# FordyceLab/magnify

Measured on AMD Instinct MI355X. Metric: megapixels/sec through flatfield+segment+ROI-reduce; markers/sec, higher is better.
Workload: dtype u16

## Files before the change

magnify_amd/csrc/mg_circles.hip:

```cpp
#include <math.h>
#include <stdlib.h>

#include "mg_common.h"

namespace {

constexpr int NT = 256;

constexpr uint64_t GOLDEN = 0x9E3779B97F4A7C15ull;
__device__ __forceinline__ uint64_t mix64(uint64_t z) {
  z ^= z >> 30;
  z *= 0xBF58476D1CE4E5B9ull;
  z ^= z >> 27;
  z *= 0x94D049BB133111EBull;
  return z ^ (z >> 31);
}
__device__ __forceinline__ uint32_t mix_top32(uint64_t z) { return (uint32_t)(mix64(z) >> 32); }

__device__ __forceinline__ uint32_t div_f64(double x, double d, double inv_d) {
  uint32_t q = (uint32_t)(x * inv_d);
  const double r = fma(-(double)q, d, x);
  if (r < 0.0) --q;
  else if (r >= d) ++q;
  return q;
}

__device__ __forceinline__ uint64_t div_u64(uint64_t n, uint64_t d, double inv_d) {
  uint64_t q = (uint64_t)((double)n * inv_d);
  int64_t r = (int64_t)(n - q * d);
  if (r < 0) {
    --q;
    r += (int64_t)d;
  }
  if (r >= (int64_t)d) ++q;
  return q;
}

constexpr double BISECTOR_EPS = (double)1e-20f;
__device__ __forceinline__ double2 bisector(int d_row, int d_col) {
  const double m = (double)(-d_col) / ((double)d_row + BISECTOR_EPS);
  return make_double2(m, 0.5 * (double)d_row - m * (0.5 * (double)d_col));
}

struct DivFull {
  __device__ __forceinline__ double operator()(double num, double den) const { return num / den; }
};
struct DivUnscaled {
  __device__ __forceinline__ double operator()(double num, double den) const {
    if (!(fabs(den) > 0.0 && fabs(den) < 1.0e300)) return num / den;
    double y = __builtin_amdgcn_rcp(den);
    double e = fma(-den, y, 1.0);
    y = fma(y, e, y);
    e = fma(-den, y, 1.0);
    y = fma(y, e, y);
    double q = num * y;
    const double r = fma(-den, q, num);
    return fma(r, y, q);
  }
};

template <class Div>
__device__ __forceinline__ float3 circle_from_bisectors(double2 l1, double2 l2, int p0r, int p0c, Div div) {
  const float c_col = (float)div(l1.y - l2.y, l2.x - l1.x + BISECTOR_EPS);
  const float c_row = (float)(l1.x * (double)c_col + l1.y);
  const float rad = sqrtf(c_row * c_row + c_col * c_col);
  return make_float3((float)((double)c_row + (double)p0r), (float)((double)c_col + (double)p0c), rad);
}

__device__ __forceinline__ void store_raw(float* __restrict__ d_raw, int64_t index, float3 c) {
  if (!d_raw) return;
  float* o = d_raw + index * 3;
  o[0] = c.x;
  o[1] = c.y;
  o[2] = c.z;
}

template <class Emit>
__device__ __forceinline__ void candidate_cell(float3 c, int h, int w, int min_r, int max_r, int ntc, Emit&& emit) {
  if (!(c.z >= (float)min_r && c.z <= (float)max_r)) return;
  const float rr = rintf(c.x), rc = rintf(c.y);
  if (!(fabsf(rr) < 1.0e9f && fabsf(rc) < 1.0e9f)) return;
  const int ir = (int)rr, ic = (int)rc, irad = (int)rintf(c.z);
  if (ir + irad < 0 || ic + irad < 0 || ir - irad >= h || ic - irad >= w) return;
  const int pr = ir + max_r, pc = ic + max_r;
  emit((pr >> 6) * ntc + (pc >> 6), irad - min_r, pr & 63, pc & 63);
}

template <bool FAST>
__global__ __launch_bounds__(NT) void k_candidates(const int32_t* __restrict__ d_coords, int64_t coord_cap,
                                                   const int32_t* __restrict__ d_starts,
                                                   const int32_t* __restrict__ d_counts,
                                                   const int32_t* __restrict__ d_num_edges, int h, int w, int grid,
                                                   int gc, int n_cells, const uint64_t* __restrict__ d_seeds,
                                                   int64_t num_iter, int min_r, int max_r,
                                                   uint32_t* __restrict__ d_bitmap, int64_t bitmap_words,
                                                   float* __restrict__ d_raw, uint32_t* __restrict__ d_keys) {
  const int plane = blockIdx.y;
  const uint32_t n_edges = (uint32_t)d_num_edges[plane];
  if (n_edges == 0) return;
  const int32_t* coords = d_coords + (int64_t)plane * coord_cap * 2;
  const int32_t* starts = d_starts + (int64_t)plane * n_cells;
  const int32_t* counts = d_counts + (int64_t)plane * n_cells;
  const uint64_t seed = d_seeds[plane];
  const int ntc = (w + 2 * max_r + 63) >> 6, nr = max_r - min_r + 1;
  uint32_t* bitmap = d_bitmap ? d_bitmap + (int64_t)plane * bitmap_words : nullptr;
  uint32_t* keys = d_keys ? d_keys + (int64_t)plane * num_iter : nullptr;
  const double inv_iter = 1.0 / (double)num_iter;
  const int64_t it0 = (int64_t)blockIdx.x * NT + threadIdx.x, stride = (int64_t)gridDim.x * NT;
  uint64_t zbase = seed + ((uint64_t)it0 * 3ull + 1ull) * GOLDEN;
  const uint64_t zstep = (uint64_t)stride * 3ull * GOLDEN;
  const uint32_t eq = FAST ? n_edges / (uint32_t)num_iter : 0u;
  const double er = FAST ? (double)(n_edges - eq * (uint32_t)num_iter) : 0.0, dk = (double)num_iter;
  const uint32_t gmagic = grid > 1 ? 0xFFFFFFFFu / (uint32_t)grid + 1u : 0u;
  for (int64_t it = it0; it < num_iter; it += stride, zbase += zstep) {
    uint64_t sa, sb;
    if (FAST) {
      const double x = (double)(uint32_t)it * er;
      sa = (uint64_t)((uint32_t)it * eq + div_f64(x, dk, inv_iter));
      sb = (uint64_t)(((uint32_t)it + 1u) * eq + div_f64(x + er, dk, inv_iter));
    } else {
      sa = div_u64((uint64_t)it * n_edges, (uint64_t)num_iter, inv_iter);
      sb = div_u64(((uint64_t)it + 1) * n_edges, (uint64_t)num_iter, inv_iter);
    }
    const uint64_t width = sb > sa ? sb - sa : 1;
    const uint32_t u0 = (uint32_t)(sa + (((uint64_t)mix_top32(zbase) * width) >> 32));
    const int p0r = coords[2 * (int64_t)u0], p0c = coords[2 * (int64_t)u0 + 1];
    const int cell = FAST ? (int)(__umulhi((uint32_t)p0r, gmagic) * (uint32_t)gc + __umulhi((uint32_t)p0c, gmagic))
                           : (p0r / grid) * gc + (p0c / grid);
    const uint32_t cnt = (uint32_t)counts[cell];
    const int64_t base = starts[cell];
    const uint64_t z12 = mix64(zbase + GOLDEN);
    const int64_t i1 = base + (int64_t)__umulhi((uint32_t)(z12 >> 32), cnt);
    const int64_t i2 = base + (int64_t)__umulhi((uint32_t)z12, cnt);
    const double2 l1 = bisector(coords[2 * i1] - p0r, coords[2 * i1 + 1] - p0c);
    const double2 l2 = bisector(coords[2 * i2] - p0r, coords[2 * i2 + 1] - p0c);
    const float3 c = circle_from_bisectors(l1, l2, p0r, p0c, DivFull{});
    store_raw(d_raw, (int64_t)plane * num_iter + it, c);
    uint32_t key = MG_NO_KEY;
    candidate_cell(c, h, w, min_r, max_r, ntc, [&](int tile, int layer, int row, int col) {
      if (keys) {
        key = mg_key_pack(tile, layer, row, col);
      } else {
        const int64_t bit = (((int64_t)tile * nr + layer) << 12) + (row << 6) + col;
        atomicOr(&bitmap[bit >> 5], 1u << (bit & 31));
      }
    });
    if (keys) keys[it] = key;
  }
}

constexpr int CT = 1024;
constexpr int MAX_TAB_GRID = 32;

__global__ __launch_bounds__(CT) void k_candidates_tab(const int32_t* __restrict__ d_coords, int64_t coord_cap,
                                                       const int32_t* __restrict__ d_starts,
                                                       const int32_t* __restrict__ d_counts,
                                                       const int32_t* __restrict__ d_num_edges, int h, int w, int grid,
                                                       int gc, int n_cells, const uint64_t* __restrict__ d_seeds,
                                                       uint32_t num_iter, int min_r, int max_r,
                                                       float* __restrict__ d_raw, uint32_t* __restrict__ d_keys) {
  extern __shared__ double2 s_tab[];
  const int plane = blockIdx.y;
  const uint32_t n_edges = (uint32_t)d_num_edges[plane];
  if (n_edges == 0) return;
  const int g1 = grid - 1, span = 2 * grid - 1;
  for (int i = threadIdx.x; i < span * span; i += CT) s_tab[i] = bisector(i / span - g1, i - (i / span) * span - g1);
  __syncthreads();
  const int32_t* coords = d_coords + (int64_t)plane * coord_cap * 2;
  const int32_t* starts = d_starts + (int64_t)plane * n_cells;
  const int32_t* counts = d_counts + (int64_t)plane * n_cells;
  const uint64_t seed = d_seeds[plane];
  const int ntc = (w + 2 * max_r + 63) >> 6;
  uint32_t* keys = d_keys ? d_keys + (int64_t)plane * num_iter : nullptr;
  const uint32_t K = num_iter;
  const uint32_t it0 = blockIdx.x * CT + threadIdx.x, stride = gridDim.x * CT;
  if (it0 >= K) return;
  const uint32_t eq = n_edges / K, er = n_edges - eq * K;
  const double inv_k = 1.0 / (double)K;
  const uint64_t x0 = (uint64_t)it0 * er;
  const uint64_t q0 = div_u64(x0, K, inv_k);
  uint32_t sa = it0 * eq + (uint32_t)q0, rem = (uint32_t)(x0 - q0 * K);
  const uint64_t xs = (uint64_t)stride * er;
  const uint64_t qs = div_u64(xs, K, inv_k);
  const uint32_t sa_step = stride * eq + (uint32_t)qs, rem_step = (uint32_t)(xs - qs * K);
  uint64_t zbase = seed + ((uint64_t)it0 * 3ull + 1ull) * GOLDEN;
  const uint64_t zstep = (uint64_t)stride * 3ull * GOLDEN;
  const uint32_t gmagic = 0xFFFFFFFFu / (uint32_t)grid + 1u;
  for (uint32_t it = it0; it < K; it += stride, zbase += zstep) {
    const uint32_t sb = sa + eq + (rem + er >= K ? 1u : 0u);
    uint32_t u0 = sa;
    if (sb > sa + 1u) u0 = sa + __umulhi(mix_top32(zbase), sb - sa);
    {
      const uint32_t t = rem + rem_step;
      const bool carry = t >= K;
      sa += sa_step + (carry ? 1u : 0u);
      rem = carry ? t - K : t;
    }
    const int2 p0 = reinterpret_cast<const int2*>(coords)[u0];
    const int p0r = p0.x, p0c = p0.y;
    const int cell = (int)(__umulhi((uint32_t)p0r, gmagic) * (uint32_t)gc + __umulhi((uint32_t)p0c, gmagic));
    const uint32_t cnt = (uint32_t)counts[cell];
    const uint32_t base = (uint32_t)starts[cell];
    const uint64_t z12 = mix64(zbase + GOLDEN);
    const uint32_t i1 = base + __umulhi((uint32_t)(z12 >> 32), cnt);
    const uint32_t i2 = base + __umulhi((uint32_t)z12, cnt);
    const int2 p1 = reinterpret_cast<const int2*>(coords)[i1], p2 = reinterpret_cast<const int2*>(coords)[i2];
    const int d1r = p1.x - p0r, d1c = p1.y - p0c, d2r = p2.x - p0r, d2c = p2.y - p0c;
    double2 l1, l2;
    if ((uint32_t)(d1r + g1) < (uint32_t)span && (uint32_t)(d1c + g1) < (uint32_t)span &&
        (uint32_t)(d2r + g1) < (uint32_t)span && (uint32_t)(d2c + g1) < (uint32_t)span) {
      l1 = s_tab[(d1r + g1) * span + d1c + g1], l2 = s_tab[(d2r + g1) * span + d2c + g1];
    } else {
      l1 = bisector(d1r, d1c), l2 = bisector(d2r, d2c);
    }
    const float3 c = circle_from_bisectors(l1, l2, p0r, p0c, DivUnscaled{});
    store_raw(d_raw, ((int64_t)plane * num_iter + it), c);
    uint32_t key = MG_NO_KEY;
    candidate_cell(c, h, w, min_r, max_r, ntc, [&](int tile, int layer, int row, int col) { key = mg_key_pack(tile, layer, row, col); });
    if (keys) keys[it] = key;
  }
}

constexpr int TS = 64;
constexpr int LAYER_WORDS = 128;

__global__ __launch_bounds__(NT) void k_layer_count(const uint32_t* __restrict__ d_bitmap, int64_t bitmap_words,
                                                    int n_layers, int32_t* __restrict__ d_layer_offsets) {
  const int plane = blockIdx.y;
  const int layer = blockIdx.x * (NT / 64) + (threadIdx.x >> 6);
  if (layer >= n_layers) return;
  const int lane = threadIdx.x & 63;
  const uint2 v = reinterpret_cast<const uint2*>(d_bitmap + (int64_t)plane * bitmap_words +
                                                 (int64_t)layer * LAYER_WORDS)[lane];
  const int c = mg_wave_sum_i32(__popc(v.x) + __popc(v.y));
  if (lane == 0) d_layer_offsets[(int64_t)plane * (n_layers + 1) + layer] = c;
}

constexpr int MAX_RANGES = 64;
constexpr int DEDUP_TX = 2;

template <int TX>
__global__ __launch_bounds__(NT) void k_tile_dedup(const uint32_t* __restrict__ d_keys, int64_t num_iter,
                                                   const int32_t* __restrict__ d_starts,
                                                   const int32_t* __restrict__ d_counts,
                                                   const int32_t* __restrict__ d_num_edges, int h, int w, int grid,
                                                   int gr, int gc, int ntc, int nr, int max_r,
                                                   uint32_t* __restrict__ d_ukeys, int64_t circle_cap,
                                                   int32_t* __restrict__ d_tile_ranges, int n_tiles,
                                                   int32_t* __restrict__ d_num_circles,
                                                   int32_t* __restrict__ d_layer_starts) {
  extern __shared__ uint32_t lbits[];
  __shared__ long long s_lo[MAX_RANGES];
  __shared__ int s_pre[MAX_RANGES + 1];
  __shared__ int s_cnt[TX * 32 + 1];
  __shared__ int s_base;
  const int plane = blockIdx.z, tr = blockIdx.y, tc0 = blockIdx.x * TX;
  const int ntx = min(TX, ntc - tc0);
  const int tile0 = tr * ntc + tc0;
  const int words = nr * LAYER_WORDS;
  for (int i = threadIdx.x; i < ntx * words; i += NT) lbits[i] = 0u;
  const long long n_edges = d_num_edges[plane];
  const int reach = max_r + 2;
  const int y0 = max(tr * TS - max_r - reach, 0), y1 = min(tr * TS + TS - 1 - max_r + reach, h - 1);
  const int x0 = max(tc0 * TS - max_r - reach, 0), x1 = min((tc0 + ntx) * TS - 1 - max_r + reach, w - 1);
  int n_ranges = 0;
  if (n_edges > 0 && y0 <= y1 && x0 <= x1) {
    const int cr0 = y0 / grid, cr1 = y1 / grid, cc0 = x0 / grid, cc1 = x1 / grid;
    n_ranges = cr1 - cr0 + 1;
    if ((int)threadIdx.x < n_ranges) {
      const int32_t* starts = d_starts + (int64_t)plane * gr * gc;
      const int32_t* counts = d_counts + (int64_t)plane * gr * gc;
      const int cr = cr0 + threadIdx.x;
      const long long ea = starts[cr * gc + cc0], eb = (long long)starts[cr * gc + cc1] + counts[cr * gc + cc1];
      long long lo = 0, hi = 0;
      if (eb > ea) {
        const double kpe = (double)num_iter / (double)n_edges;
        hi = min((long long)((double)eb * kpe) + 3, (long long)num_iter);
        lo = min(max((long long)((double)ea * kpe) - 2, 0ll), hi);
      }
      s_lo[threadIdx.x] = lo;
      s_pre[threadIdx.x + 1] = (int)(hi - lo);
    }
  }
  __syncthreads();
  if (threadIdx.x == 0) {
    s_pre[0] = 0;
    for (int r = 0; r < n_ranges; ++r) s_pre[r + 1] += s_pre[r];
  }
  __syncthreads();
  const uint32_t* keys = d_keys + (int64_t)plane * num_iter;
  constexpr int KB = 8;
  for (int r = 0; r < n_ranges; ++r) {
    const uint32_t* kr = keys + s_lo[r];
    const int len = s_pre[r + 1] - s_pre[r];
    for (int base = threadIdx.x; base < len; base += NT * KB) {
      uint32_t kv[KB];
#pragma unroll
      for (int u = 0; u < KB; ++u) {
        const int i = base + u * NT;
        kv[u] = i < len ? kr[i] : MG_NO_KEY;
      }
#pragma unroll
      for (int u = 0; u < KB; ++u) {
        const uint32_t key = kv[u];
        const uint32_t t = mg_key_tile(key) - (uint32_t)tile0;
        if (t < (uint32_t)ntx) atomicOr(&lbits[t * words + (mg_key_low17(key) >> 5)], 1u << (key & 31u));
      }
    }
  }
  __syncthreads();
  const int n_li = ntx * nr;
  const int n_words = n_li * LAYER_WORDS;
  const int per = (n_words + NT - 1) / NT;
  const int w0 = min((int)threadIdx.x * per, n_words), w1 = min(w0 + per, n_words);
  int mine = 0;
  for (int wd = w0; wd < w1; ++wd) mine += __popc(lbits[wd]);
  int n_unique;
  const int ex = mg_block_exscan(mine, &n_unique);
  {
    int run = ex;
    for (int wd = w0; wd < w1; ++wd) {
      if ((wd & (LAYER_WORDS - 1)) == 0) s_cnt[wd / LAYER_WORDS] = run;
      run += __popc(lbits[wd]);
    }
  }
  if (threadIdx.x == 0) {
    s_cnt[n_li] = n_unique;
    s_base = n_unique ? atomicAdd(&d_num_circles[plane], n_unique) : 0;
  }
  __syncthreads();
  const int64_t base = s_base;
  if ((int)threadIdx.x < ntx) {
    int32_t* tr2 = d_tile_ranges + ((int64_t)plane * n_tiles + tile0 + threadIdx.x) * 2;
    tr2[0] = (int32_t)min(base + s_cnt[threadIdx.x * nr], circle_cap);
    tr2[1] = s_cnt[(threadIdx.x + 1) * nr] - s_cnt[threadIdx.x * nr];
  }
  if (d_layer_starts) {
    for (int i = threadIdx.x; i < ntx * (nr + 1); i += NT) {
      const int t = i / (nr + 1), ri = i - t * (nr + 1);
      d_layer_starts[((int64_t)plane * n_tiles + tile0 + t) * (nr + 1) + ri] =
          (int32_t)min(base + s_cnt[t * nr + ri], circle_cap);
    }
  }
  uint32_t* out = d_ukeys + (int64_t)plane * circle_cap;
  int64_t pos = base + ex;
  for (int wd = w0; wd < w1; ++wd) {
    uint32_t bits = lbits[wd];
    if (!bits) continue;
    int t = 0, rem = wd;
#pragma unroll
    for (int k = 1; k < TX; ++k)
      if (rem >= words) rem -= words, ++t;
    const uint32_t hi = mg_key_from_low17(tile0 + t, (uint32_t)rem << 5);
    while (bits) {
      const int b = __ffs(bits) - 1;
      bits &= bits - 1;
      if (pos < circle_cap) out[pos] = hi | (uint32_t)b;
      ++pos;
    }
  }
}

__global__ __launch_bounds__(1024) void k_layer_scan(int32_t* __restrict__ d_layer_offsets, int n_layers,
                                                     int32_t* __restrict__ d_num_circles, int64_t cap) {
  const int plane = blockIdx.x;
  int32_t* cnt = d_layer_offsets + (int64_t)plane * (n_layers + 1);
  const int per = (n_layers + 1023) / 1024;
  const int lo = min((int)threadIdx.x * per, n_layers), hi = min(lo + per, n_layers);
  int sum = 0;
  for (int i = lo; i < hi; ++i) sum += cnt[i];
  int total;
  int run = mg_block_exscan(sum, &total);
  for (int i = lo; i < hi; ++i) {
    const int v = cnt[i];
    cnt[i] = run;
    run += v;
  }
  if (threadIdx.x == 0) {
    cnt[n_layers] = total;
    d_num_circles[plane] = (int32_t)min((int64_t)total, cap);
  }
}

__global__ __launch_bounds__(NT) void k_layer_emit(uint32_t* __restrict__ d_bitmap, int64_t bitmap_words, int n_layers,
                                                   const int32_t* __restrict__ d_layer_offsets, int ntc, int nr,
                                                   int min_r, int max_r, int32_t* __restrict__ d_circles,
                                                   int64_t circle_cap) {
  const int plane = blockIdx.y;
  const int layer = blockIdx.x * (NT / 64) + (threadIdx.x >> 6);
  if (layer >= n_layers) return;
  const int lane = threadIdx.x & 63;
  const int32_t* lo = d_layer_offsets + (int64_t)plane * (n_layers + 1);
  if (lo[layer + 1] == lo[layer]) return;
  uint2* words = reinterpret_cast<uint2*>(d_bitmap + (int64_t)plane * bitmap_words + (int64_t)layer * LAYER_WORDS);
  const uint2 v = words[lane];
  uint64_t bits = ((uint64_t)v.y << 32) | v.x;
  if (bits) words[lane] = make_uint2(0u, 0u);
  const int c = __popcll(bits);
  int incl = c;
#pragma unroll
  for (int off = 1; off < 64; off <<= 1) {
    const int t = __shfl_up(incl, off);
    if (lane >= off) incl += t;
  }
  int64_t pos = (int64_t)lo[layer] + incl - c;
  const int tile = layer / nr, ri = layer - tile * nr;
  const int row = (tile / ntc) * TS + lane - max_r, col0 = (tile % ntc) * TS - max_r;
  int32_t* out = d_circles + (int64_t)plane * circle_cap * 3;
  while (bits) {
    const int b = __ffsll((unsigned long long)bits) - 1;
    bits &= bits - 1;
    if (pos < circle_cap) {
      out[3 * pos] = row;
      out[3 * pos + 1] = col0 + b;
      out[3 * pos + 2] = min_r + ri;
    }
    ++pos;
  }
}

__device__ __forceinline__ uint32_t bits_at(const uint32_t* __restrict__ bits, int64_t bit0, int n) {
  const int64_t wi = bit0 >> 5;
  const int sh = (int)(bit0 & 31);
  uint64_t two = bits[wi];
  if (sh + n > 32) two |= (uint64_t)bits[wi + 1] << 32;
  const uint32_t v = (uint32_t)(two >> sh);
  return n >= 32 ? v : (v & ((1u << n) - 1u));
}

__device__ __forceinline__ int32_t per_pack(int dr, int quarter, int dc) { return (dr << 16) | (quarter << 14) | (dc & 0x3FFF); }
__device__ __forceinline__ int per_dr(int32_t v) { return v >> 16; }
__device__ __forceinline__ int per_dc(int32_t v) { return ((int)((uint32_t)v << 18)) >> 18; }
__device__ __forceinline__ int per_quarter(int32_t v) { return (v >> 14) & 3; }

constexpr int CHUNK = 1024;
constexpr int SURV_IDX_BITS = 20;

template <int WS, bool KEYED>
__global__ __launch_bounds__(NT) __attribute__((amdgpu_num_sgpr(96))) void k_score_tiles(const float* __restrict__ d_angle,
                                                    const uint32_t* __restrict__ d_bits,
                                                    const uint32_t* __restrict__ d_class, int64_t words_per_plane,
                                                    int h, int w, int32_t* __restrict__ d_circles,
                                                    int64_t circle_cap, const int32_t* __restrict__ d_layer_offsets,
                                                    const uint32_t* __restrict__ d_ukeys,
                                                    const int32_t* __restrict__ d_tile_ranges, int n_tiles,
                                                    int n_layers, int nr, int ntc, int min_r, int max_r,
                                                    const int32_t* __restrict__ d_per_rc, int per_total,
                                                    const double* __restrict__ d_per_expected,
                                                    const int32_t* __restrict__ d_per_starts, float min_roundness,
                                                    int write_skipped, int dedup_centres,
                                                    float* __restrict__ d_scores,
                                                    int32_t* __restrict__ d_alive, int32_t* __restrict__ d_num_alive,
                                                    int32_t* __restrict__ d_max_rc, int32_t* __restrict__ d_num_scored) {
  extern __shared__ uint32_t lds[];
  __shared__ int n_surv, n_pass;
  const int plane = blockIdx.y, tile = blockIdx.x;
  int64_t first, last;
  if (KEYED) {
    const int32_t* tr2 = d_tile_ranges + ((int64_t)plane * n_tiles + tile) * 2;
    first = tr2[0];
    last = min(first + tr2[1], circle_cap);
  } else {
    const int32_t* lo = d_layer_offsets + (int64_t)plane * (n_layers + 1);
    first = lo[(int64_t)tile * nr];
    last = min((int64_t)lo[(int64_t)(tile + 1) * nr], circle_cap);
  }
  if (first >= last) return;
  const int side = TS + 2 * max_r;
  int wsh = 0;
  while ((32 << wsh) < side) ++wsh;
  const int wpr = 1 << wsh;
  const int slot = WS ? WS : side * wpr;
  uint32_t* win = lds;
  int32_t* tab = reinterpret_cast<int32_t*>(lds + 4 * slot);
  int32_t* list = tab + per_total;
  const int wy0 = (tile / ntc) * TS - 2 * max_r, wx0 = (tile % ntc) * TS - 2 * max_r;
  const uint32_t* bits = d_bits + plane * words_per_plane;
  const uint32_t* cls0 = d_class ? d_class + (3 * plane) * words_per_plane : nullptr;
  const uint32_t* cls1 = d_class ? d_class + (3 * plane + 1) * words_per_plane : nullptr;
  for (int i = threadIdx.x; i < side * wpr; i += NT) {
    const int j = i >> wsh, k = i & (wpr - 1);
    const int y = wy0 + j, xs = wx0 + 32 * k;
    uint32_t v = 0, c0 = 0, c1 = 0;
    if (y >= 0 && y < h) {
      const int x_lo = max(xs, 0), x_hi = min(min(xs + 32, wx0 + side), w);
      if (x_lo < x_hi) {
        v = bits_at(bits, (int64_t)y * w + x_lo, x_hi - x_lo) << (x_lo - xs);
        if (d_class && v) {
          c0 = bits_at(cls0, (int64_t)y * w + x_lo, x_hi - x_lo) << (x_lo - xs);
          c1 = bits_at(cls1, (int64_t)y * w + x_lo, x_hi - x_lo) << (x_lo - xs);
        }
      }
    }
    if (d_class) {
      win[i] = v & ~(c1 & ~c0);
      win[slot + i] = v & ~(c1 & c0);
      win[2 * slot + i] = v & (c1 | c0);
      win[3 * slot + i] = v & (c1 | ~c0);
    } else {
      win[i] = win[slot + i] = win[2 * slot + i] = win[3 * slot + i] = v;
    }
  }
  for (int i = threadIdx.x; i < per_total; i += NT) {
    const int dr = d_per_rc[2 * i], dc = d_per_rc[2 * i + 1];
    const int ay = abs(dr), ax = abs(dc);
    const int quarter = ((dr ^ dc) < 0) ? (ay > ax ? 2 : 3) : (ay < ax ? 0 : 1);
    tab[i] = per_pack(dr, quarter, dc);
  }
  __syncthreads();
  int32_t* circles = d_circles + (int64_t)plane * circle_cap * 3;
  const uint32_t* ukeys = KEYED ? d_ukeys + (int64_t)plane * circle_cap : nullptr;
  const int trow0 = (tile / ntc) * TS - max_r, tcol0 = (tile % ntc) * TS - max_r;
  struct Circle {
    int row, col, rad;
  };
  auto load_circle = [&](int64_t i) -> Circle {
    if constexpr (KEYED) {
      const uint32_t key = ukeys[i];
      return {trow0 + mg_key_row(key), tcol0 + mg_key_col(key), min_r + mg_key_layer(key)};
    } else {
      return {circles[3 * i], circles[3 * i + 1], circles[3 * i + 2]};
    }
  };
  const float* ang = d_angle + (int64_t)plane * h * w;
  float* scores = d_scores + (int64_t)plane * circle_cap;
  constexpr int BATCH = 2 * NT;
  constexpr int PASS_CAP = 64, SURV_ROOM = CHUNK - 3 * PASS_CAP;
  if (threadIdx.x == 0) n_pass = 0;
  for (int64_t chunk = first; chunk < last;) {
    if (threadIdx.x == 0) n_surv = 0;
    __syncthreads();
    int64_t pos = chunk;
    for (;;) {
    for (int64_t i = pos + threadIdx.x; i < min(pos + BATCH, last); i += NT) {
      const auto [row, col, rad] = load_circle(i);
      const int p0 = d_per_starts[rad - min_r], p1 = d_per_starts[rad - min_r + 1];
      const int need = (int)ceil(mg_score_floor(min_roundness, p1 - p0));
      const int by = row - wy0, bx = col - wx0;
      auto bit = [&](const uint32_t* ww, int yy, int xx) -> uint32_t {
        return (ww[((by + yy) << wsh) + ((bx + xx) >> 5)] >> ((bx + xx) & 31)) & 1u;
      };
      const uint32_t *w0 = win, *w1 = win + slot, *w2 = win + 2 * slot, *w3 = win + 3 * slot;
      int hits = bit(w3, 0, -rad) + bit(w2, -rad, 0) + bit(w0, 0, rad) + bit(w1, rad, 0);
      int p = p0 + 4;
      for (; p + 8 <= p1; p += 8) {
        const int v = tab[p];
        const int x = per_dr(v), y = per_dc(v);
        hits += bit(w3, x, y) + bit(w2, y, x) + bit(w0, -x, y) + bit(w1, -y, x) + bit(w0, x, -y) +
                bit(w1, y, -x) + bit(w3, -x, -y) + bit(w2, -y, -x);
      }
      if (p + 4 == p1) {
        const int v = tab[p];
        const int x = per_dr(v), y = per_dc(v);
        const uint32_t* wa = win + (((x ^ y) < 0) ? 3 : 1) * slot;
        const uint32_t* wb = win + (((x ^ y) < 0) ? 1 : 3) * slot;
        hits += bit(wa, x, y) + bit(wa, -x, -y) + bit(wb, -x, y) + bit(wb, x, -y);
      }
      if (hits >= need) {
        list[atomicAdd(&n_surv, 1)] = (int32_t)(i - chunk) | (hits << SURV_IDX_BITS);
      } else if (write_skipped) {
        scores[i] = MG_SCORE_SKIPPED;
      }
    }
      pos += BATCH;
      __syncthreads();
      const int so_far = n_surv;
      if (pos >= last || so_far > SURV_ROOM - BATCH || pos - chunk > (1 << SURV_IDX_BITS) - BATCH) break;
      __syncthreads();
    }
    const int ns = n_surv;
    if (threadIdx.x == 0 && d_num_scored) atomicAdd(&d_num_scored[plane], ns);
    for (int a = threadIdx.x; a < ns; a += NT) {
      const int64_t i = chunk + (list[a] & ((1 << SURV_IDX_BITS) - 1));
      const auto [row, col, rad] = load_circle(i);
      const int p0 = d_per_starts[rad - min_r], p1 = d_per_starts[rad - min_r + 1];
      const int by = row - wy0, bx = col - wx0;
      double acc = 0.0;
      double left = (double)(list[a] >> SURV_IDX_BITS);
      const double floor_sum = mg_score_floor(min_roundness, p1 - p0);
      bool dead = false;
      for (int base = p0; base < p1 && !dead; base += 32) {
        uint32_t mask = 0, counted = 0;
        const int cnt = min(32, p1 - base);
        for (int j = 0; j < cnt; ++j) {
          const int v = tab[base + j];
          const int y = by + per_dr(v), x = bx + per_dc(v);
          const int wi = (y << wsh) + (x >> 5);
          mask |= (((win[wi] | win[2 * slot + wi]) >> (x & 31)) & 1u) << j;
          counted |= ((win[per_quarter(v) * slot + wi] >> (x & 31)) & 1u) << j;
        }
        constexpr int PF = 8;
        while (mask && !dead) {
          int jj[PF];
          float an[PF];
#pragma unroll
          for (int u = 0; u < PF; ++u) {
            jj[u] = __ffs(mask) - 1;
            mask &= mask - 1;
            an[u] = 0.0f;
            if (jj[u] >= 0) {
              const int v = tab[base + jj[u]];
              an[u] = ang[(int64_t)(__umul24(row + per_dr(v), w) + (col + per_dc(v)))];
            }
          }
#pragma unroll
          for (int u = 0; u < PF; ++u) {
            if (jj[u] < 0 || dead) continue;
            const int p = base + jj[u];
            acc += mg_alignment_term(an[u], d_per_expected[p]);
            left -= (double)((counted >> jj[u]) & 1u);
            if (acc + left < floor_sum) dead = true;
          }
        }
      }
      if (dead) {
        if (write_skipped) scores[i] = MG_SCORE_SKIPPED;
        continue;
      }
      const float score = (float)acc / (float)(p1 - p0);
      scores[i] = score;
      if (score >= min_roundness) {
        const int slot = dedup_centres ? atomicAdd(&n_pass, 1) : PASS_CAP;
        if (slot < PASS_CAP) {
          list[CHUNK - 1 - 3 * slot] = (int32_t)(i - first);
          list[CHUNK - 2 - 3 * slot] = __float_as_int(score);
          list[CHUNK - 3 - 3 * slot] = (int32_t)mg_key_pack(0, rad, row - trow0, col - tcol0);
        } else {
          mg_emit_alive<KEYED>(d_num_alive, d_alive, d_max_rc, plane, circle_cap, circles, i, row, col, rad);
        }
      }
    }
    __syncthreads();
    chunk = pos;
  }
  const int np = min(n_pass, PASS_CAP);
  for (int a = threadIdx.x; a < np; a += NT) {
    const int code = list[CHUNK - 3 - 3 * a];
    const float score = __int_as_float(list[CHUNK - 2 - 3 * a]);
    bool first_at_centre = true;
    for (int b = 0; b < np; ++b) {
      const int code_b = list[CHUNK - 3 - 3 * b];
      const float score_b = __int_as_float(list[CHUNK - 2 - 3 * b]);
      if (((code ^ code_b) & MG_KEY_CENTRE_MASK) == 0 && (score_b > score || (score_b == score && code_b < code))) first_at_centre = false;
    }
    if (first_at_centre) {
      const int64_t i = first + list[CHUNK - 1 - 3 * a];
      mg_emit_alive<KEYED>(d_num_alive, d_alive, d_max_rc, plane, circle_cap, circles, i, trow0 + mg_key_row(code),
                           tcol0 + mg_key_col(code), code >> MG_KEY_LAYER_SHIFT);
    }
  }
}

__device__ __forceinline__ uint32_t nms_sort_bits(float score) {
  uint32_t b = __float_as_uint(score);
  b = (b & 0x80000000u) ? ~b : (b | 0x80000000u);
  return ~b;
}
__device__ __forceinline__ uint64_t nms_key(float score, uint32_t idx) { return ((uint64_t)nms_sort_bits(score) << 32) | idx; }

__device__ __forceinline__ int wrap(int v, int n) {
  if (v >= n) {
    v -= n;
    if (v >= n) v %= n;
// ... 722 lines not shown
```

Baseline: 215,600.

## Single-pass bitmap scan with nonempty-word mask and packed key writes in tile dedup

The tile-dedup kernel now reads each thread's run of shared bitmap words once, recording the popcount, the prefix at the layer boundary and a 32-bit mask of non-empty words. The second and third passes over shared memory go away. Key emission walks only the non-empty words through the mask and writes keys in groups of four. Block indexing is also remapped so that consecutive blocks go to different planes. Risks are the misaligned 16-byte stores through Keys4 and the static assumption that a thread's run fits in 32 words.

```diff
diff --git a/magnify_amd/csrc/mg_circles.hip b/magnify_amd/csrc/mg_circles.hip
--- a/magnify_amd/csrc/mg_circles.hip
+++ b/magnify_amd/csrc/mg_circles.hip
@@ -238,6 +238,9 @@
 
 constexpr int MAX_RANGES = 64;
 constexpr int DEDUP_TX = 2;
+struct Keys4 {
+  uint32_t k[4];
+};
 
 template <int TX>
 __global__ __launch_bounds__(NT) void k_tile_dedup(const uint32_t* __restrict__ d_keys, int64_t num_iter,
@@ -254,7 +257,9 @@
   __shared__ int s_pre[MAX_RANGES + 1];
   __shared__ int s_cnt[TX * 32 + 1];
   __shared__ int s_base;
-  const int plane = blockIdx.z, tr = blockIdx.y, tc0 = blockIdx.x * TX;
+  const int lin = blockIdx.x + gridDim.x * (blockIdx.y + gridDim.y * blockIdx.z);
+  const int plane = lin % (int)gridDim.z, group = lin / (int)gridDim.z;
+  const int tr = group / (int)gridDim.x, tc0 = (group - tr * (int)gridDim.x) * TX;
   const int ntx = min(TX, ntc - tc0);
   const int tile0 = tr * ntc + tc0;
   const int words = nr * LAYER_WORDS;
@@ -309,21 +314,27 @@
     }
   }
   __syncthreads();
+  static_assert(TX * 32 * LAYER_WORDS <= 32 * NT, "a thread's run of words must fit the 32-bit mask of non-empty words");
   const int n_li = ntx * nr;
   const int n_words = n_li * LAYER_WORDS;
   const int per = (n_words + NT - 1) / NT;
   const int w0 = min((int)threadIdx.x * per, n_words), w1 = min(w0 + per, n_words);
-  int mine = 0;
-  for (int wd = w0; wd < w1; ++wd) mine += __popc(lbits[wd]);
+  const int wb = (w0 + LAYER_WORDS - 1) & ~(LAYER_WORDS - 1);
+  const int n_run = w1 - w0, j_start = wb - w0;
+  const uint32_t* run = lbits + w0;
+  int mine = 0, head = 0;
+  uint32_t full = 0u;
+#pragma clang loop vectorize(disable)
+#pragma unroll 4
+  for (int j = 0; j < n_run; ++j) {
+    const uint32_t v = run[j];
+    head = j == j_start ? mine : head;
+    mine += __popc(v);
+    full |= min(v, 1u) << j;
+  }
   int n_unique;
   const int ex = mg_block_exscan(mine, &n_unique);
-  {
-    int run = ex;
-    for (int wd = w0; wd < w1; ++wd) {
-      if ((wd & (LAYER_WORDS - 1)) == 0) s_cnt[wd / LAYER_WORDS] = run;
-      run += __popc(lbits[wd]);
-    }
-  }
+  if (wb < w1) s_cnt[wb / LAYER_WORDS] = ex + head;
   if (threadIdx.x == 0) {
     s_cnt[n_li] = n_unique;
     s_base = n_unique ? atomicAdd(&d_num_circles[plane], n_unique) : 0;
@@ -343,22 +354,31 @@
     }
   }
   uint32_t* out = d_ukeys + (int64_t)plane * circle_cap;
-  int64_t pos = base + ex;
-  for (int wd = w0; wd < w1; ++wd) {
-    uint32_t bits = lbits[wd];
-    if (!bits) continue;
-    int t = 0, rem = wd;
-#pragma unroll
-    for (int k = 1; k < TX; ++k)
-      if (rem >= words) rem -= words, ++t;
-    const uint32_t hi = mg_key_from_low17(tile0 + t, (uint32_t)rem << 5);
-    while (bits) {
-      const int b = __ffs(bits) - 1;
-      bits &= bits - 1;
-      if (pos < circle_cap) out[pos] = hi | (uint32_t)b;
-      ++pos;
-    }
-  }
+  const int64_t first = min(base + ex, circle_cap);
+  const int room = (int)min((int64_t)mine, circle_cap - first);
+  uint32_t* mykeys = out + first;
+  const uint32_t key0 = mg_key_from_low17(tile0, 0u), next_tile = mg_key_from_low17(1, 0u) - ((uint32_t)words << 5);
+  uint32_t bits = 0u, hi = 0u;
+  auto next_key = [&]() -> uint32_t {
+    if (!bits) {
+      const int wd = w0 + __builtin_ctz(full);
+      full &= full - 1;
+      bits = lbits[wd];
+      hi = key0 + ((uint32_t)wd << 5);
+#pragma unroll
+      for (int t = 1; t < TX; ++t) hi += wd >= t * words ? next_tile : 0u;
+    }
+    const uint32_t key = hi | (uint32_t)__builtin_ctz(bits);
+    bits &= bits - 1;
+    return key;
+  };
+  int k = 0;
+  for (; k + 4 <= room; k += 4) {
+    Keys4 q;
+    q.k[0] = next_key(), q.k[1] = next_key(), q.k[2] = next_key(), q.k[3] = next_key();
+    *reinterpret_cast<Keys4*>(mykeys + k) = q;
+  }
+  for (; k < room; ++k) mykeys[k] = next_key();
 }
 
 __global__ __launch_bounds__(1024) void k_layer_scan(int32_t* __restrict__ d_layer_offsets, int n_layers,
```

After: 225,400 (median of 6 runs). 4.6% higher.
